# twosigma/Cook

Measured on AMD Instinct MI355X. Metric: match-cycles/sec at 1M pending x 50k offers, higher is better.
Workload: dtype f64

## Files before the change

### cook_amd/csrc/rank_host.hpp

```cpp

template <class T, class Load>
void seg_scan(cook_engine* e, const char* tag, Load load, const uint8_t* head, unsigned n, T* out, ScanTmp<T>& tmp) {
  if (n == 0) return;
  const unsigned nb = div_up(n, SS_TILE);
  tmp.agg.ensure(nb);
  tmp.carry.ensure(nb);
  tmp.first_head.ensure(nb);
  KM<seg_scan_local<T, Load>, SS_THREADS>(e, tag, nb, load, head, n, out, tmp.agg.ptr(), tmp.first_head.ptr());
  if (nb > 1 && nb <= (unsigned)SS_THREADS) {
    KM<seg_scan_propagate_fused<T>, SS_THREADS>(e, "seg_scan_propagate", nb, out, n, (const SegAgg<T>*)tmp.agg.ptr(), (const unsigned*)tmp.first_head.ptr());
  } else if (nb > 1) {
    KM<seg_scan_blocksums<T>, SS_THREADS>(e, "seg_scan_blocksums", 1, (const SegAgg<T>*)tmp.agg.ptr(), nb, tmp.carry.ptr());
    KM<seg_scan_propagate<T>, SS_THREADS>(e, "seg_scan_propagate", nb, out, n, (const SegAgg<T>*)tmp.carry.ptr(), (const unsigned*)tmp.first_head.ptr());
  }
}

template <int IPL>
static void radix_pass_t(cook_engine* e, const uint64_t* key, const uint32_t* in, uint32_t* out, unsigned n, unsigned shift, bool fused,
                         DArr<uint32_t>& hist) {
  const unsigned nb = div_up(n, rs_tile(IPL));
  hist.ensure((size_t)256 * nb);
  KM<radix_hist<IPL>, RS_THREADS>(e, "radix_hist", nb, key, in, n, shift, nb, fused ? 1u : 0u, hist.ptr());
  if (!fused) KM<excl_scan_u32_single, SCAN1_THREADS>(e, "radix_scan", 1, hist.ptr(), 256u * nb, (uint32_t*)nullptr);
  KM<radix_scatter<IPL>, RS_THREADS>(e, "radix_scatter", nb, key, in, out, n, shift, nb, fused ? 1u : 0u, (const uint32_t*)hist.ptr());
}
void radix_pass(cook_engine* e, const uint64_t* key, const uint32_t* in, uint32_t* out, unsigned n, unsigned shift, DArr<uint32_t>& hist) {
  if (div_up(n, rs_tile(RS_IPL_SMALL)) <= RS_FUSED_BLOCKS) radix_pass_t<RS_IPL_SMALL>(e, key, in, out, n, shift, true, hist);
  else radix_pass_t<RS_IPL_LARGE>(e, key, in, out, n, shift, div_up(n, rs_tile(RS_IPL_LARGE)) <= RS_FUSED_BLOCKS_LARGE, hist);
}
uint32_t* radix_sort_masked(cook_engine* e, const uint64_t* key, unsigned long long mask, const uint32_t* cur, uint32_t* a,
                            uint32_t* b, unsigned n, DArr<uint32_t>* hist = nullptr) {
  const uint32_t* in = cur;
  uint32_t* last = const_cast<uint32_t*>(cur);
  while (mask) {
    const unsigned shift = (unsigned)__builtin_ctzll(mask);
    uint32_t* out = (in == a) ? b : a;
    radix_pass(e, key, in, out, n, shift, hist ? *hist : e->hist);
    in = out;
    last = out;
    mask = shift + 8 >= 64 ? 0ull : mask & ~((1ull << (shift + 8)) - 1ull);
  }
  return last;
}

COOK_KERNEL void iota_u32(uint32_t* p, unsigned n) {
  const unsigned i = blockIdx.x * blockDim.x + threadIdx.x;
  if (i < n) p[i] = i;
}

void rank_stage(cook_engine* e, const cook_tasks* t, const cook_users* u) {
  if (!t || !u) e->fail(COOK_E_INVALID, "cook_rank_stage: null tasks/users");
  const unsigned N = t->n, U = u->n;
  if (N && (!t->cpus || !t->mem || !t->user || !t->priority || !t->start_ms || !t->task_id || !t->job_id || !t->pending))
    e->fail(COOK_E_INVALID, "cook_rank_stage: a required task array is NULL");
  if (U == 0 && N) e->fail(COOK_E_INVALID, "cook_rank_stage: no users");
  unsigned np = 0;
  std::vector<uint32_t> pend_ord(N ? N : 1);
  for (unsigned i = 0; i < N; ++i) {
    if (t->user[i] >= U) e->fail(COOK_E_INVALID, "cook_rank_stage: user id out of range");
    pend_ord[i] = np;
    np += t->pending[i] ? 1u : 0u;
  }
  e->rank_staged = false, e->pool_usage_known = false, e->rank_done = false;
  e->N = N;
  e->U = U;
  e->n_pending = np;
  e->has_gpus = t->gpus != nullptr;
  h2d(e, e->t_cpus, t->cpus, N);
  h2d(e, e->t_mem, t->mem, N);
  if (t->gpus) h2d(e, e->t_gpus, t->gpus, N);
  h2d(e, e->t_user, t->user, N);
  h2d(e, e->t_prio, t->priority, N);
  h2d(e, e->t_start, t->start_ms, N);
// ... 365 lines not shown
```

### cook_amd/csrc/sort.hpp

```cpp
#pragma once
#include "common.hpp"

constexpr int RS_THREADS = 256;
constexpr int RS_WAVES = RS_THREADS / COOK_WAVE;
constexpr int RS_IPL_LARGE = 16;
constexpr int RS_IPL_SMALL = 8;
constexpr unsigned RS_FUSED_BLOCKS = COOK_SHAPE(128, 2);
constexpr unsigned RS_FUSED_BLOCKS_LARGE = COOK_SHAPE(512, 3);
constexpr unsigned rs_tile(int ipl) { return (unsigned)(RS_WAVES * COOK_WAVE * ipl); }

static __device__ __forceinline__ unsigned rs_digit(const uint64_t* __restrict__ key, const uint32_t* __restrict__ perm_in,
                                                    unsigned i, unsigned shift) {
  const unsigned src = perm_in ? perm_in[i] : i;
  return (unsigned)(key[src] >> shift) & 0xFFu;
}

template <int IPL>
COOK_KERNEL void radix_hist(const uint64_t* __restrict__ key, const uint32_t* __restrict__ perm_in,
                                                         unsigned n, unsigned shift, unsigned nblocks, unsigned fused,
                                                         uint32_t* __restrict__ hist) {
  __shared__ unsigned h[256];
  h[threadIdx.x] = 0;
  __syncthreads();
  const unsigned base = blockIdx.x * rs_tile(IPL);
// ... 43 lines not shown
      for (int q = 0; q < SCAN1_IPT; ++q) tot += v[s][q];
      unsigned inc = tot;
      for (unsigned d = 1; d < COOK_WAVE; d <<= 1) {
        const unsigned t = __shfl_up(inc, d, COOK_WAVE);
        if (lane >= d) inc += t;
      }
      if (lane == COOK_WAVE - 1) wsum[s & 1][w] = inc;
      __syncthreads();
      unsigned wbase = 0, all = 0;
      for (unsigned k = 0; k < SCAN1_THREADS / COOK_WAVE; ++k) {
        const unsigned x = wsum[s & 1][k];
        wbase += k < w ? x : 0u;
        all += x;
      }
      unsigned run = carry + wbase + inc - tot;
      unsigned o[SCAN1_IPT];
#pragma unroll
      for (int q = 0; q < SCAN1_IPT; ++q) {
        o[q] = run;
        run += v[s][q];
      }
      if (i0 + SCAN1_IPT <= len) {
        *reinterpret_cast<uint4*>(data + i0) = uint4{o[0], o[1], o[2], o[3]};
        *reinterpret_cast<uint4*>(data + i0 + 4) = uint4{o[4], o[5], o[6], o[7]};
      } else {
#pragma unroll
        for (int q = 0; q < SCAN1_IPT; ++q)
          if (i0 + q < len) data[i0 + q] = o[q];
      }
      carry += all;
    }
  }
  if (total_out && threadIdx.x == 0) *total_out = carry;
}

template <int IPL>
COOK_KERNEL void radix_scatter(const uint64_t* __restrict__ key, const uint32_t* __restrict__ perm_in,
                                                            uint32_t* __restrict__ perm_out, unsigned n, unsigned shift,
                                                            unsigned nblocks, unsigned fused, const uint32_t* __restrict__ hist) {
  __shared__ unsigned whist[RS_WAVES][256];
  __shared__ unsigned wtot[RS_WAVES];
  __shared__ uint4 s_tot[RS_WAVES][COOK_WAVE], s_bel[RS_WAVES][COOK_WAVE];
  const unsigned lane = lane_id(), w = wave_id();
  for (int k = 0; k < RS_WAVES; ++k) whist[k][threadIdx.x] = 0;
  unsigned below = 0, total = 0;
  if (fused) {
    uint4 tot{0u, 0u, 0u, 0u}, bel{0u, 0u, 0u, 0u};
#pragma unroll 8
    for (unsigned t = w; t < nblocks; t += RS_WAVES) {
      const uint4 v = *reinterpret_cast<const uint4*>(hist + (size_t)t * 256u + 4u * lane);
      tot.x += v.x, tot.y += v.y, tot.z += v.z, tot.w += v.w;
      if (t < blockIdx.x) bel.x += v.x, bel.y += v.y, bel.z += v.z, bel.w += v.w;
    }
    s_tot[w][lane] = tot;
    s_bel[w][lane] = bel;
  }
  __syncthreads();
  if (fused) {
    const unsigned* pt = reinterpret_cast<const unsigned*>(&s_tot[0][0]);
    const unsigned* pb = reinterpret_cast<const unsigned*>(&s_bel[0][0]);
    for (int k = 0; k < RS_WAVES; ++k) {
      total += pt[k * 256 + threadIdx.x];
      below += pb[k * 256 + threadIdx.x];
    }
  }
  const unsigned wbase = blockIdx.x * rs_tile(IPL) + w * (COOK_WAVE * IPL);
// ... 2 lines not shown
  for (int k = 0; k < IPL; ++k) {
    const unsigned i = wbase + k * COOK_WAVE + lane;
    src[k] = i < n ? (perm_in ? perm_in[i] : i) : 0xFFFFFFFFu;
  }
#pragma unroll
  for (int k = 0; k < IPL; ++k) dg[k] = src[k] != 0xFFFFFFFFu ? (unsigned)(key[src[k]] >> shift) & 0xFFu : 0u;
#pragma unroll
  for (int k = 0; k < IPL; ++k)
    if (src[k] != 0xFFFFFFFFu) atomicAdd(&whist[w][dg[k]], 1u);
  if (fused) {
    unsigned inc = total;
    for (unsigned d = 1; d < COOK_WAVE; d <<= 1) {
      const unsigned t = __shfl_up(inc, d, COOK_WAVE);
      if (lane >= d) inc += t;
    }
    if (lane == COOK_WAVE - 1) wtot[w] = inc;
    __syncthreads();
    unsigned before = 0;
    for (unsigned k = 0; k < (unsigned)RS_WAVES; ++k) before += k < w ? wtot[k] : 0u;
    below += before + inc - total;
  } else {
    __syncthreads();
    below = hist[threadIdx.x * nblocks + blockIdx.x];
  }
  {
    unsigned base = below;
    for (int k = 0; k < RS_WAVES; ++k) {
      const unsigned t = whist[k][threadIdx.x];
      whist[k][threadIdx.x] = base;
      base += t;
    }
  }
  __syncthreads();
  const unsigned long long lt = lanemask_lt();
#pragma unroll
  for (int k = 0; k < IPL; ++k) {
    const bool valid = src[k] != 0xFFFFFFFFu;
    const unsigned d = dg[k];
    unsigned long long peers = __ballot(valid);
    for (int b = 0; b < 8; ++b) {
      const unsigned long long m = __ballot(valid && ((d >> b) & 1u));
      peers &= ((d >> b) & 1u) ? m : ~m;
    }
    unsigned slot = 0;
    if (valid) slot = whist[w][d];
    wave_sync();
    if (valid) {
      const unsigned rank = (unsigned)__popcll(peers & lt);
      if (rank == 0) whist[w][d] = slot + (unsigned)__popcll(peers);
      perm_out[slot + rank] = src[k];
    }
    wave_sync();
  }
}

COOK_KERNEL void radix_varying_bits(const uint64_t* __restrict__ key, unsigned n,
                                                          unsigned long long* __restrict__ out_mask, unsigned nblk) {
  const uint64_t k0 = key[0];
  unsigned long long m = 0;
  for (unsigned i = blockIdx.x * blockDim.x + threadIdx.x; i < n; i += nblk * blockDim.x) m |= key[i] ^ k0;
  for (int d = 32; d >= 1; d >>= 1) m |= __shfl_xor(m, d, COOK_WAVE);
  __shared__ unsigned long long s_m[256 / COOK_WAVE];
  if (lane_id() == 0) s_m[wave_id()] = m;
  __syncthreads();
  if (threadIdx.x == 0) {
    unsigned long long b = 0ull;
    for (unsigned w = 0; w < blockDim.x / COOK_WAVE; ++w) b |= s_m[w];
    if (b) atomicOr(out_mask, b);
  }
}
```

### cook_amd/csrc/classfit_walk.hpp

```cpp
#pragma once
#if defined(CF_PROF) && !defined(CF_STATS)
#define CF_STATS 1
#endif
#ifdef CF_STATS
#define CF_STAT(x) x
#define CF_TICKS() cook_ticks()
#else
#define CF_STAT(x) ((void)0)
#define CF_TICKS() 0ull
#endif
#ifdef CF_PROF
#define CF_PROF_T(x) const unsigned long long x = __builtin_readcyclecounter()
#define CF_PROF_ADD(i, d) prof[i] += (unsigned long long)(d)
#else
#define CF_PROF_T(x) ((void)0)
#define CF_PROF_ADD(i, d) ((void)0)
#endif

#ifndef CF_AHEAD
#define CF_AHEAD 10
#endif
constexpr unsigned CF_BOARD = CF_AHEAD;
#ifndef CF_SLOTS_N
#define CF_SLOTS_N 12
// ... 23 lines not shown
  uint32_t ofc, ofm, nfc, nfm, pad0, pad1;
};
struct CfPost {
  double fa;
  uint32_t w0;
  uint32_t pos;
  uint32_t fc, fm, cls, aux;
};
struct CfJobU {
  unsigned c, m, kind, L, n_eq, n_nov, grouped, grp, eq0, eq1, nov0, nov1;
};
struct CfLds {
  CfFree* fcm;
  uint16_t* cid;
  CfEnt* board;
  CfLog* log;
  uint32_t* ctrl;
  uint64_t* attr8;
  uint16_t *goff, *gcnt, *gids;
  CfJob* ring;
  CfPost* post2;
  CfClass* cls;
  uint32_t* pw;
  uint32_t* aw;
  uint32_t* gk;
  uint32_t* ovt;
  uint32_t* ovl;
  uint32_t* ckept;
  uint32_t* misc;
  const uint32_t* t;
  const uint32_t* envw;
};

static __device__ __forceinline__ unsigned cf_level_of(const uint32_t* t, uint32_t fc) {
  unsigned n = 0;
#pragma unroll
  for (int i = 0; i < CF_LV; ++i) n += fc >= t[i] ? 1u : 0u;
  return n;
}
struct CfLv8 {
  uint32_t v0, v1, v2, v3, v4, v5, v6, v7;
};
#define CF_FOR8(F) F(0) F(1) F(2) F(3) F(4) F(5) F(6) F(7)
static __device__ __forceinline__ uint32_t cf_lv_get(const CfLv8& a, unsigned i) {
  const bool b0 = (i & 1u) != 0u, b1 = (i & 2u) != 0u, b2 = (i & 4u) != 0u;
  const uint32_t r01 = b0 ? a.v1 : a.v0, r23 = b0 ? a.v3 : a.v2, r45 = b0 ? a.v5 : a.v4, r67 = b0 ? a.v7 : a.v6;
  const uint32_t r03 = b1 ? r23 : r01, r47 = b1 ? r67 : r45;
  return b2 ? r47 : r03;
}
struct CfChunkLane {
  unsigned cls, kind, pos0, n, Tc, Tm;
  unsigned long long dE;
  double hTc, hTm;
  CfLv8 lv, la;
};

static __device__ __forceinline__ void cf_setup_chunks(const CfClass* cls, unsigned nc, unsigned lw, unsigned lane, CfChunkLane& c, unsigned& nch_wave) {
  c.cls = 0xFFu, c.kind = 0xFEu, c.pos0 = 0u, c.n = 0u, c.Tc = 1u, c.Tm = 1u, c.dE = 0ull, c.hTc = 0.0, c.hTm = 0.0;
  unsigned acc = 0;
  for (unsigned ci = 0; ci < nc; ++ci) {
    const CfClass& cl = cls[ci];
    if (cl.wave != lw) continue;
    const unsigned nch = (cl.n + 63u) / 64u;
    if (lane >= acc && lane < acc + nch) {
      const unsigned x = lane - acc;
      c.cls = ci, c.kind = cl.kind, c.pos0 = cl.off + 64u * x, c.n = cf_min(64u, cl.n - 64u * x), c.Tc = cl.Tc, c.Tm = cl.Tm, c.dE = cl.dE, c.hTc = cl.hTc, c.hTm = cl.hTm;
    }
    acc += nch;
  }
  nch_wave = acc;
}

static __device__ __forceinline__ void cf_tighten(const CfLds& S, unsigned lane, unsigned ch, CfChunkLane& c) {
  const uint32_t* t = S.t;
  const unsigned pos0 = (unsigned)wave_read_lane((int)c.pos0, (int)ch), n = (unsigned)wave_read_lane((int)c.n, (int)ch);
  const bool in = lane < n;
  const CfFree f = S.fcm[pos0 + lane];
  const uint32_t cid = S.cid[pos0 + lane];
  const unsigned nl = in ? cf_level_of(t, f.c) : 0u;
  const bool free_host = !(cid & CF_OCC);
#define CF_TI_A(i) unsigned a##i = nl > (unsigned)i ? f.m + 1u : 0u;
#define CF_TI_R(i) unsigned r##i = (nl > (unsigned)i && free_host) ? f.m + 1u : 0u;
  CF_FOR8(CF_TI_A)
  CF_FOR8(CF_TI_R)
#undef CF_TI_A
#undef CF_TI_R
  wave_max8_u32(a0, a1, a2, a3, a4, a5, a6, a7);
  wave_max8_u32(r0, r1, r2, r3, r4, r5, r6, r7);
#define CF_TI_S(i) \
  if (lane == ch) c.la.v##i = a##i, c.lv.v##i = r##i;
  CF_FOR8(CF_TI_S)
#undef CF_TI_S
}
static __device__ __forceinline__ void cf_wave_tables(const CfLds& S, unsigned lw, unsigned lane, const CfChunkLane& c, unsigned kinds, unsigned n_kind) {
#define CF_TB_P(i) unsigned p##i = c.kind == 0u ? c.lv.v##i : 0u;
#define CF_TB_A(i) unsigned a##i = c.kind < 0xFEu ? c.la.v##i : 0u;
  CF_FOR8(CF_TB_P)
  CF_FOR8(CF_TB_A)
#undef CF_TB_P
#undef CF_TB_A
  wave_max8_u32(p0, p1, p2, p3, p4, p5, p6, p7);
  wave_max8_u32(a0, a1, a2, a3, a4, a5, a6, a7);
#define CF_TB_S(i) \
  if (lane == 0) S.pw[lw * CF_LV + i] = p##i, S.aw[lw * CF_LV + i] = a##i;
  CF_FOR8(CF_TB_S)
#undef CF_TB_S
  for (unsigned k = 1; k < n_kind; ++k) {
    if (!((kinds >> k) & 1u)) continue;
#define CF_TB_G(i) unsigned g##i = c.kind == k ? c.lv.v##i : 0u;
    CF_FOR8(CF_TB_G)
#undef CF_TB_G
    wave_max8_u32(g0, g1, g2, g3, g4, g5, g6, g7);
#define CF_TB_GS(i) \
  if (lane == 0) S.gk[k * CF_LV + i] = g##i;
    CF_FOR8(CF_TB_GS)
#undef CF_TB_GS
  }
}

static __device__ __forceinline__ bool cf_cons_ok(const CfLds& S, const CfJobU& J, unsigned id, bool active) {
  bool ok = true;
  if (J.n_eq) {
    const uint64_t a8 = S.attr8[active ? id : 0u];
#pragma unroll
    for (unsigned q = 0; q < 4u; ++q) {
      const unsigned e = ((q < 2u ? J.eq0 : J.eq1) >> (16u * (q & 1u))) & 0xFFFFu;
      if (q < J.n_eq) ok = ok && (unsigned)((a8 >> (8u * (e >> 8))) & 255ull) == (e & 255u);
    }
  }
  if (J.n_nov) {
#pragma unroll
    for (unsigned q = 0; q < 4u; ++q) {
      const unsigned h = ((q < 2u ? J.nov0 : J.nov1) >> (16u * (q & 1u))) & 0xFFFFu;
      if (q < J.n_nov) ok = ok && id != h;
    }
  }
  if (J.grouped) {
    const unsigned g0 = S.goff[J.grp], gn = ld_wg(&S.gcnt[J.grp]);
    for (unsigned x = 0; x < gn; ++x) ok = ok && id != (unsigned)S.gids[g0 + x];
  }
  return ok;
}
static __device__ __forceinline__ double cf_literal(unsigned Tc, unsigned Tm, unsigned fc, unsigned fm, unsigned jc, unsigned jm, double sc, double sm) {
  const double A = (double)(Tc - fc) * sc, Bm = (double)(Tm - fm) * sm, c = (double)jc * sc, m = (double)jm * sm;
  return ((A + c) / ((double)Tc * sc) + (Bm + m) / ((double)Tm * sm)) / 2.0;
}

struct CfAns {
  bool have, amb;
  unsigned pos, ch, cid, fc, fm, cls;
  double fa;
};
static __device__ __forceinline__ void cf_class_answer(const CfLds& S, const CfJobU& J, unsigned lane, CfChunkLane& c, CfAns& out, unsigned& scans,
                                                       unsigned& tightened) {
  out.have = false, out.amb = false, out.pos = 0u, out.ch = 0u, out.cid = 0u, out.fc = 0u, out.fm = 0u, out.cls = 0u, out.fa = 0.0;
  const uint32_t lvL = cf_lv_get(c.lv, J.L);
  unsigned long long m = __ballot(c.kind == J.kind && lvL > J.m);
  while (m) {
    const unsigned ch = (unsigned)__ffsll(m) - 1u;
    ++scans;
    const unsigned pos0 = (unsigned)wave_read_lane((int)c.pos0, (int)ch), n = (unsigned)wave_read_lane((int)c.n, (int)ch);
    const unsigned q = pos0 + lane;
    const CfFree f = S.fcm[q];
    const uint32_t cid = S.cid[q];
    const bool room = lane < n && f.c >= J.c && f.m >= J.m && !(cid & CF_OCC);
    const bool ok = room && cf_cons_ok(S, J, cid & CF_IDMASK, room);
    const unsigned long long b = __ballot(ok);
    if (b == 0ull) {
      if (__ballot(room) == 0ull) {
        cf_tighten(S, lane, ch, c);
        ++tightened;
      }
      m &= ~(1ull << ch);
      continue;
    }
    const unsigned q0 = (unsigned)__ffsll(b) - 1u;
    const unsigned fc0 = (unsigned)wave_read_lane((int)f.c, (int)q0), fm0 = (unsigned)wave_read_lane((int)f.m, (int)q0), cid0 = (unsigned)wave_read_lane((int)cid, (int)q0);
    const unsigned cls = (unsigned)wave_read_lane((int)c.cls, (int)ch);
    m &= ~__ballot(c.cls == cls);
    const bool tie = (cid0 & CF_TIE) != 0u;
    const double hTc = wave_read_lane_f64(c.hTc, (int)ch), hTm = wave_read_lane_f64(c.hTm, (int)ch);
    const double f0 = 1.0 - ((double)(fc0 - J.c) * hTc + (double)(fm0 - J.m) * hTm);
    if (!out.have || f0 > out.fa + CF_BAND) out.amb = tie;
    else if (f0 >= out.fa - CF_BAND) out.amb = true;
    if (!out.have || f0 > out.fa) out.fa = f0, out.cid = cid0 & CF_IDMASK, out.pos = pos0 + q0, out.fc = fc0, out.fm = fm0, out.cls = cls, out.ch = ch;
    out.have = true;
  }
}
static __device__ __forceinline__ void cf_class_query_exact(const CfLds& S, const CfJobU& J, unsigned lane, const CfChunkLane& c, double fmax, double sc, double sm, CfPost& out,
                                                            unsigned& scans) {
  out.fa = 0.0, out.w0 = 0u, out.pos = 0u, out.fc = 0u, out.fm = 0u, out.cls = 0u, out.aux = 0u;
  const uint32_t lvL = cf_lv_get(c.lv, J.L);
  unsigned long long m = __ballot(c.kind == J.kind && lvL > J.m);
  unsigned long long best_lit = 0ull;
  while (m) {
    const unsigned ch = (unsigned)__ffsll(m) - 1u;
    ++scans;
    const unsigned pos0 = (unsigned)wave_read_lane((int)c.pos0, (int)ch), n = (unsigned)wave_read_lane((int)c.n, (int)ch);
    const unsigned Tc = (unsigned)wave_read_lane((int)c.Tc, (int)ch), Tm = (unsigned)wave_read_lane((int)c.Tm, (int)ch), cls = (unsigned)wave_read_lane((int)c.cls, (int)ch);
    const double hTc = wave_read_lane_f64(c.hTc, (int)ch), hTm = wave_read_lane_f64(c.hTm, (int)ch);
    const unsigned q = pos0 + lane;
    const CfFree f = S.fcm[q];
    const uint32_t cid = S.cid[q];
// ... 48 lines not shown
  const bool has = lane == 0u || (lane < 7u && ((used_sets >> lane) & 1u));
  CfPost p;
  p.fa = 0.0, p.w0 = 0u, p.pos = p.fc = p.fm = p.cls = p.aux = 0u;
  if (has) p = posts[lane];
  const unsigned long long fb = (unsigned long long)__double_as_longlong(p.fa);
  const unsigned long long mx = wave_max_u64(fb);
  v.src = -1, v.id = v.pos = v.fc = v.fm = v.cls = v.aux = 0u;
  if (mx == 0ull) return v;
  const unsigned idmin = ~wave_max_u32((has && fb == mx) ? ~p.w0 : 0u);
  const unsigned wl = (unsigned)__ffsll(__ballot(has && fb == mx && p.w0 == idmin)) - 1u;
  v.src = (int)wl;
  v.id = (unsigned)wave_read_lane((int)p.w0, (int)wl), v.pos = (unsigned)wave_read_lane((int)p.pos, (int)wl), v.fc = (unsigned)wave_read_lane((int)p.fc, (int)wl),
  v.fm = (unsigned)wave_read_lane((int)p.fm, (int)wl), v.cls = (unsigned)wave_read_lane((int)p.cls, (int)wl), v.aux = (unsigned)wave_read_lane((int)p.aux, (int)wl);
  return v;
}
static __device__ __forceinline__ unsigned cf_poll(const uint32_t* p) { return (unsigned)wave_read_lane((int)ld_wg(p), 0); }
static __device__ __forceinline__ unsigned long long cf_below(unsigned s) { return (1ull << s) - 1ull; }

enum : unsigned { CFE_K = 0, CFE_M, CFE_NP, CFE_NCLS, CFE_NKIND, CFE_CMIN, CFE_MMIN, CFE_KC, CFE_KM, CFE_MINFC, CFE_MINFM, CFE_N = 12 };
constexpr float CF_BAND32 = 1.0f / 2097152.0f;

struct CfFixed {
  CfEnt board[CF_SLOTS * 8u];
  CfLog log[64];
  CfJob ring[2u * 64u];
  CfPost post2[8];
  CfClass cls[CF_MAXCLS];
  uint32_t pw[8u * CF_LV], aw[8u * CF_LV], gk[CF_MAXKIND * CF_LV], ovt[CF_LV];
  uint32_t ctrl[8];
  uint32_t ovl[192], ckept[3u * CF_MAXCLS], misc[CFX_N];
  uint32_t env_t[CF_LV], envw[CFE_N];
};
static_assert(sizeof(CfFixed) % 16 == 0, "the arrays behind it are 16-byte aligned");
#if COOK_HAS_ASM_WALK
#define CF_ASM_EPOCH_LIVE "57"
#include "classfit_asm.hpp"
static_assert(CF_EPOCH_AT == 58 && CF_OVL == 58, "classfit_asm.hpp: the overlay's size");
static_assert(offsetof(CfFixed, ctrl) == 13728 + (CF_SLOTS - 12) * 256 && offsetof(CfFixed, cls) == 9472 + (CF_SLOTS - 12) * 256 && sizeof(CfFixed) == 15280 + (CF_SLOTS - 12) * 256 && sizeof(CfClass) == 56 && offsetof(CfClass, hTc) == 32 &&
                  offsetof(CfClass, hTm) == 40 && offsetof(CfEnt, pos) == 8 && offsetof(CfEnt, cid) == 12 && offsetof(CfEnt, fc) == 16 && offsetof(CfEnt, fa) == 24 && sizeof(CfEnt) == 32 &&
                  sizeof(CfLog) == 32 && offsetof(CfLog, ofc) == 8,
              "classfit_asm.hpp: offsets of the LDS records");
typedef unsigned cf_u32x16 __attribute__((ext_vector_type(16)));
typedef unsigned cf_u32x8 __attribute__((ext_vector_type(8)));
typedef unsigned cf_u32x4 __attribute__((ext_vector_type(4)));
#endif

template <int ROLE>
static __device__ __forceinline__ void cf_walk_role(const CfLds& S, const MatchState& st, const CfBuf& b, const unsigned lw, const unsigned rep, const unsigned nrep,
                                                    const unsigned long long t_start) {
  constexpr bool is_decider = ROLE == 0, is_class_wave = ROLE == 1, is_books = ROLE == 2;
  const unsigned tid = threadIdx.x, lane = lane_id();
  CfCtl* ctl = b.ctl;
  const unsigned K = wave_uniform_u32(S.envw[CFE_K]), cmin = wave_uniform_u32(S.envw[CFE_CMIN]), mmin = wave_uniform_u32(S.envw[CFE_MMIN]);
  const uint32_t* t = S.t;
#define n_cls wave_uniform_u32(S.envw[CFE_NCLS])
#define n_kind wave_uniform_u32(S.envw[CFE_NKIND])
#define NP wave_uniform_u32(S.envw[CFE_NP])
  CfChunkLane c;
  unsigned nch_wave = 0;
  cf_setup_chunks(S.cls, n_cls, is_class_wave ? lw : 0xFFu, lane, c, nch_wave);
  c.lv = CfLv8{0u, 0u, 0u, 0u, 0u, 0u, 0u, 0u}, c.la = c.lv;
  unsigned my_kinds = 0;
  {
    const unsigned forw = is_class_wave ? lw : (is_decider && lane >= CF_OVL ? lane - CF_OVL + 1u : 0xFFu);
    for (unsigned ci = 0; ci < n_cls; ++ci)
      if (S.cls[ci].wave == forw && S.cls[ci].kind < 32u) my_kinds |= 1u << S.cls[ci].kind;
  }
  const unsigned wk = is_class_wave ? wave_uniform_u32(my_kinds) : 0u;
  unsigned one_cls = 0xFFFFFFFFu, u_off = 0, u_n = 0;
  double u_hTc = 0.0, u_hTm = 0.0;
  auto class_setup = [&] {
    unsigned cnt = 0, ci0 = 0;
    for (unsigned ci = 0; ci < n_cls; ++ci)
      if (S.cls[ci].wave == lw) ++cnt, ci0 = ci;
    one_cls = cnt == 1u ? ci0 : 0xFFFFFFFFu;
    const CfClass* cl = &S.cls[ci0];
    u_off = cl->off, u_n = cl->n, u_hTc = cl->hTc, u_hTm = cl->hTm;
  };
  if (is_class_wave) {
    class_setup();
    for (unsigned ch = 0; ch < nch_wave; ++ch) cf_tighten(S, lane, ch, c);
    if (rep == 0u && lw != 0u) cf_wave_tables(S, lw, lane, c, wk, n_kind);
  }
  CfOvLane o;
  o.valid = 0u, o.id = 0u, o.cls = 0u, o.fc = 0u, o.fm = 0u, o.hTc = 0.0, o.hTm = 0.0;
  unsigned nrm = 0, rm1 = 0xFFFFFFFFu, rm2 = 0xFFFFFFFFu;
  unsigned minfc_all = wave_uniform_u32(S.envw[CFE_MINFC]), minfm_all = wave_uniform_u32(S.envw[CFE_MINFM]);
  unsigned matched = 0, head = 0;
  unsigned jc = 0, jm = 0, jmeta = 0, jgrp = 0, jeq0 = 0, jeq1 = 0, jnov0 = 0, jnov1 = 0;
  int res = -1;
  unsigned long long b1m = 0ull;
  unsigned seen = 0, gen = 0;
  unsigned tight_applied = 0;
  bool bk_room0 = false, nx_room0 = false, nx_walk = false;
  unsigned st_scans = 0, st_exact = 0, st_open = 0, st_ovwin = 0, st_gpu = 0, st_epochs = 0, st_tight = 0, st_walked = 0, st_dead = 0, st_opendead = 0, st_spins = 0, st_flips = 0,
           st_rewinds = 0;
  unsigned long long tk_epoch = 0, tk_books = 0, tk_walk = 0, tk_phase1 = 0;
#ifdef CF_PROF
  unsigned long long prof[8] = {0, 0, 0, 0, 0, 0, 0, 0}, bnd0 = 0ull;
#endif
  auto job_of = [&](unsigned s) -> CfJobU {
    CfJobU J;
    J.c = (unsigned)wave_read_lane((int)jc, (int)s), J.m = (unsigned)wave_read_lane((int)jm, (int)s);
    const unsigned meta = (unsigned)wave_read_lane((int)jmeta, (int)s);
    J.kind = meta & 255u, J.L = (meta >> 8) & 15u, J.n_eq = (meta >> 12) & 15u, J.n_nov = (meta >> 16) & 15u, J.grouped = (meta >> 20) & 1u;
    J.grp = 0u, J.eq0 = J.eq1 = 0u, J.nov0 = J.nov1 = 0xFFFFFFFFu;
    if (meta >> 12) {
      J.grp = (unsigned)wave_read_lane((int)jgrp, (int)s), J.eq0 = (unsigned)wave_read_lane((int)jeq0, (int)s), J.eq1 = (unsigned)wave_read_lane((int)jeq1, (int)s),
      J.nov0 = (unsigned)wave_read_lane((int)jnov0, (int)s), J.nov1 = (unsigned)wave_read_lane((int)jnov1, (int)s);
    }
    return J;
  };
  auto tables_room_any = [&](unsigned L, unsigned m) -> bool {
    bool r = S.ovt[L] > m;
// ... 365 lines not shown
              }
            }
            bool done = false;
            if ((meta >> 12) == 0u && one_cls != 0xFFFFFFFFu) {
              const uint32_t lvL = cf_lv_get(c.lv, (meta >> 8) & 15u);
              const unsigned long long mk = cook_ballot(lvL > Jm);
              if (mk == 0ull) {
                st_lane0_b32(&e->tag, 0xFFFFFFFFu);
                st_lane0_b64(&e->pos, 0u, CF_ENT_NONE);
                st_lane0_b32(&e->tag, tag);
                done = true;
              } else {
                const unsigned ch = (unsigned)__ffsll(mk) - 1u;
                const unsigned pos0 = u_off + 64u * ch, n = u_n - 64u * ch;
                const CfFree f = S.fcm[pos0 + lane];
                const uint32_t cid = S.cid[pos0 + lane];
                const unsigned long long bb = cook_ballot((lane < n) & (f.c >= Jc) & (f.m >= Jm) & !(cid & CF_OCC));
                double fa = 1.0 - ((double)(f.c - Jc) * u_hTc + (double)(f.m - Jm) * u_hTm);
                if (bb != 0ull) {
                  const unsigned long long pm = bb & (0ull - bb);
                  const unsigned long long fb = (unsigned long long)__double_as_longlong(fa);
                  st_mask_b32(&e->tag, pm, 0xFFFFFFFFu);
                  st_mask_b128(&e->fc, pm, f.c, f.m, (unsigned)fb, (unsigned)(fb >> 32));
                  st_mask_b64(&e->pos, pm, (pos0 + lane) | ch << 16, (cid & CF_IDMASK) | one_cls << 16 | ((cid & CF_TIE) ? CF_ENT_AMB : 0u));
                  st_mask_b32(&e->tag, pm, tag);
                  done = true;
                  CF_STAT(++st_scans);
                }
              }
            }
            if (!done) {
              const CfJobU J = job_of(s);
              CfAns a;
              cf_class_answer(S, J, lane, c, a, st_scans, st_tight);
              const unsigned long long fb = (unsigned long long)__double_as_longlong(a.fa);
              st_lane0_b32(&e->tag, 0xFFFFFFFFu);
              st_lane0_b128(&e->fc, a.fc, a.fm, (unsigned)fb, (unsigned)(fb >> 32));
              st_lane0_b64(&e->pos, a.pos | a.ch << 16, a.have ? (a.cid | a.cls << 16 | (a.amb ? CF_ENT_AMB : 0u)) : CF_ENT_NONE);
              st_lane0_b32(&e->tag, tag);
            }
            CF_PROF_T(q2);
            CF_PROF_ADD(0, q1 - q0);
            CF_PROF_ADD(1, q2 - q1);
            CF_PROF_ADD(3, 1);
          };
          if (cnt != seen) {
            seen = cnt;
            CF_STAT(++st_rewinds);
            unsigned long long t2 = walkmask & ~cf_below(hw & 255u);
            unsigned o2 = hw >> 8, p2 = o2;
            while (p2 >= nrep) p2 -= nrep;
            for (; t2 != 0ull && o2 < cur_ord; t2 &= t2 - 1ull, ++o2, p2 = p2 + 1u == nrep ? 0u : p2 + 1u)
              if (p2 == rep && wk != 0u) answer((unsigned)__ffsll(t2) - 1u, o2, true);
          }
          if (cur_ord < (hw >> 8)) {
            todo = walkmask & ~cf_below(hw & 255u);
            cur_ord = hw >> 8;
            ph = cur_ord;
            while (ph >= nrep) ph -= nrep;
          }
          while (todo != 0ull && ph != rep) {
            todo &= todo - 1ull, ++cur_ord;
            ph = ph + 1u == nrep ? 0u : ph + 1u;
          }
          if (todo != 0ull && wk != 0u && cur_ord < (hw >> 8) + CF_BOARD) {
            const unsigned s = (unsigned)__ffsll(todo) - 1u;
            const unsigned ord = cur_ord;
// ... 185 lines not shown
              }
              for (; ip < li + ni; ++ip) {
                const unsigned np = noff + kept_before + (ip - li);
                if (lane == 0) st_agent(&b.scr_fc[np], S.ovl[3u * ip + 1u]), st_agent(&b.scr_fm[np], S.ovl[3u * ip + 2u]), st_agent(&b.scr_cid[np], S.ovl[3u * ip]);
              }
            }
            li += ni;
          }
        }
        drain_stores();
        EMU_SITE("classfit: epoch 3");
        __syncthreads();
        unsigned newM = 0;
        for (unsigned ci = 0; ci < n_cls; ++ci) newM += S.ckept[ci] + S.ckept[CF_MAXCLS + ci];
        for (unsigned q = tid; q < NP; q += CF_THREADS) {
          const bool inq = q < newM;
          const uint32_t fcq = inq ? ld_agent(&b.scr_fc[q]) : 0u, fmq = inq ? ld_agent(&b.scr_fm[q]) : 0u, cq = inq ? ld_agent(&b.scr_cid[q]) : 0u;
          bool tie = false;
          if (q + 1u < newM) {
            const uint32_t fcn = ld_agent(&b.scr_fc[q + 1u]), fmn = ld_agent(&b.scr_fm[q + 1u]), cn = ld_agent(&b.scr_cid[q + 1u]);
            if ((cn >> 16) == (cq >> 16)) {
              const CfClass* cl = &S.cls[cq >> 16];
              tie = (unsigned long long)fcn * cl->Tm + (unsigned long long)fmn * cl->Tc <= (unsigned long long)fcq * cl->Tm + (unsigned long long)fmq * cl->Tc + cl->dE;
            }
          }
          S.fcm[q] = CfFree{fcq, fmq}, S.cid[q] = inq ? (uint16_t)((cq & (CF_OCC | CF_IDMASK)) | (tie ? CF_TIE : 0u)) : (uint16_t)0u;
        }
        if (tid < n_cls) S.cls[tid].n = S.ckept[tid] + S.ckept[CF_MAXCLS + tid], S.cls[tid].off = S.ckept[2 * CF_MAXCLS + tid];
        EMU_SITE("classfit: epoch 4");
        __syncthreads();
        if (is_class_wave) {
          cf_setup_chunks(S.cls, n_cls, lw, lane, c, nch_wave);
          class_setup();
          for (unsigned ch = 0; ch < nch_wave; ++ch) cf_tighten(S, lane, ch, c);
          if (rep == 0u && lw != 0u) cf_wave_tables(S, lw, lane, c, wk, n_kind);
          tight_applied = st_tight;
        }
        if (tid == 0) S.misc[CFX_LOG_APPLIED] = S.misc[CFX_LOGN];
        tk_epoch += CF_TICKS() - te;
      }
      {
        ++gen;
        if (is_class_wave) {
          todo = walkmask & ~cf_below(s) & ~(1ull << s), cur_ord = (unsigned)__popcll(walkmask & cf_below(s)) + 1u;
          ph = cur_ord;
          while (ph >= nrep) ph -= nrep;
        }
      }
      if (tid == 0) st_wg(&S.ctrl[0], 0u);
      EMU_SITE("classfit: collective done");
      __syncthreads();
      if (is_class_wave) seen = cf_poll(&S.ctrl[1u + lw]);
    }
    tk_walk += CF_TICKS() - tw0;
    CF_PROF_T(cw1);
    CF_PROF_ADD(7, cw1 - cw0);
    const unsigned long long tp0 = CF_TICKS();
    if (is_decider && nw == 0u) decider_books(0u);
    if (nw != 0u) {
      if (is_class_wave) {
        const unsigned n_log = wave_uniform_u32(S.misc[CFX_LOGN]), a0 = wave_uniform_u32(S.misc[CFX_LOG_APPLIED]);
        const bool mine_e = lane >= a0 && lane < n_log && ((S.log[lane].info >> 8) & 15u) == lw;
        bool dirty = st_tight != tight_applied;
        for (unsigned long long mm = __ballot(mine_e); mm; mm &= mm - 1ull) {
          const unsigned x = (unsigned)__ffsll(mm) - 1u;
          const CfLog lg = S.log[x];
          const unsigned ch = (lg.info >> 12) & 255u;
          bool retable = ((lg.info >> 20) & 1u) != 0u;
          const unsigned nl = cf_level_of(t, lg.ofc);
#define CF_WAS_MAX(i) retable = retable || (__ballot(lane == ch && (unsigned)i < nl && c.lv.v##i == lg.ofm + 1u) != 0ull);
          CF_FOR8(CF_WAS_MAX)
#undef CF_WAS_MAX
          if (retable) {
            cf_tighten(S, lane, ch, c);
            ++st_tight;
            dirty = true;
          }
        }
        if (dirty && rep == 0u && lw != 0u) cf_wave_tables(S, lw, lane, c, wk, n_kind);
        tight_applied = st_tight;
      }
    }
    EMU_SITE("classfit: phase 2");
    __syncthreads();
    tk_phase1 += CF_TICKS() - tp0;
    if (is_books) {
      const unsigned long long tb0 = CF_TICKS();
      const unsigned long long mm = (unsigned long long)S.misc[CFX_MATCH_LO] | (unsigned long long)S.misc[CFX_MATCH_HI] << 32,
                               bb = (unsigned long long)S.misc[CFX_B1_LO] | (unsigned long long)S.misc[CFX_B1_HI] << 32;
      const unsigned n_log = wave_uniform_u32(S.misc[CFX_LOGN]);
      const CfJob j = S.ring[slot * 64u + (lane < bn ? lane : 0u)];
      const bool unm = lane < bn && !((mm >> lane) & 1ull);
      const unsigned L = (j.meta >> 8) & 15u;
      bool room = unm && tables_room_any(L, j.m);
      const bool flip = unm && !room && bk_room0 && n_log != 0u;
      if (__ballot(flip) != 0ull) {
        ++st_flips;
        for (unsigned x = 0; x < n_log; ++x) {
          const CfLog lg = S.log[x];
          if (flip && (lg.info & 255u) > lane && lg.ofc >= j.c && lg.ofm >= j.m) room = true;
        }
      }
      if (lane < bn && st.fail_code) {
        unsigned fail = 0u;
        if (unm) {
          fail = (((bb >> lane) & 1ull) ? 1u : 0u) | (room ? 2u : 0u);
          if (fail == 0u) fail = 8u;
        }
        st.fail_code[base + lane] = fail;
      }
// ... 198 lines not shown
```

Measured before the change: 21.69.

## Add onesweep radix sort with decoupled lookback and single multi-digit histogram

```diff
diff --git a/cook_amd/csrc/rank_host.hpp b/cook_amd/csrc/rank_host.hpp
--- a/cook_amd/csrc/rank_host.hpp
+++ b/cook_amd/csrc/rank_host.hpp
@@ -19,26 +19,70 @@
 static void radix_pass_t(cook_engine* e, const uint64_t* key, const uint32_t* in, uint32_t* out, unsigned n, unsigned shift, bool fused,
                          DArr<uint32_t>& hist) {
   const unsigned nb = div_up(n, rs_tile(IPL));
-  hist.ensure((size_t)256 * nb);
-  KM<radix_hist<IPL>, RS_THREADS>(e, "radix_hist", nb, key, in, n, shift, nb, fused ? 1u : 0u, hist.ptr());
-  if (!fused) KM<excl_scan_u32_single, SCAN1_THREADS>(e, "radix_scan", 1, hist.ptr(), 256u * nb, (uint32_t*)nullptr);
-  KM<radix_scatter<IPL>, RS_THREADS>(e, "radix_scatter", nb, key, in, out, n, shift, nb, fused ? 1u : 0u, (const uint32_t*)hist.ptr());
-}
-void radix_pass(cook_engine* e, const uint64_t* key, const uint32_t* in, uint32_t* out, unsigned n, unsigned shift, DArr<uint32_t>& hist) {
-  if (div_up(n, rs_tile(RS_IPL_SMALL)) <= RS_FUSED_BLOCKS) radix_pass_t<RS_IPL_SMALL>(e, key, in, out, n, shift, true, hist);
-  else radix_pass_t<RS_IPL_LARGE>(e, key, in, out, n, shift, div_up(n, rs_tile(RS_IPL_LARGE)) <= RS_FUSED_BLOCKS_LARGE, hist);
+  uint32_t* h = hist.ptr() + RS1_OFF_STATUS;
+  KM<radix_hist<IPL>, RS_THREADS>(e, "radix_hist", nb, key, in, n, shift, nb, fused ? 1u : 0u, h);
+  if (!fused) KM<excl_scan_u32_single, SCAN1_THREADS>(e, "radix_scan", 1, h, 256u * nb, (uint32_t*)nullptr);
+  KM<radix_scatter<IPL>, RS_THREADS>(e, "radix_scatter", nb, key, in, out, n, shift, nb, fused ? 1u : 0u, (const uint32_t*)h);
+}
+COOK_KERNEL void radix_scratch_clear(uint32_t* __restrict__ p, unsigned n) {
+  const unsigned i = blockIdx.x * blockDim.x + threadIdx.x;
+  if (i < n) p[i] = 0u;
+}
+static void radix_scratch(cook_engine* e, DArr<uint32_t>& hist, size_t words) {
+  const void* was = hist.b.p;
+  const size_t cap = hist.b.cap;
+  hist.ensure(words);
+  if (hist.b.p != was || hist.b.cap != cap) KM<radix_scratch_clear, 256>(e, "radix_scratch_clear", div_up(RS1_OFF_BASE, 256), hist.ptr(), RS1_OFF_BASE);
+}
+template <int IPL>
+static void radix_onesweep_t(cook_engine* e, const uint64_t* key, const RadixDigits& dg, const uint32_t*& in, uint32_t*& last, uint32_t* a, uint32_t* b,
+                             unsigned n, DArr<uint32_t>& hist) {
+  const unsigned nb = div_up(n, rs_tile(IPL));
+  const size_t per_digit = (size_t)nb * 256u;
+  radix_scratch(e, hist, RS1_OFF_STATUS + dg.nd * per_digit);
+  uint32_t* h = hist.ptr();
+  const unsigned nblk = std::min(div_up(n, RH_TILE), RH_MAX_BLOCKS);
+  KM<radix_hist_digits, RH_THREADS>(e, "radix_hist_digits", nblk, key, n, dg, nblk, h + RS1_OFF_ACC, h + RS1_OFF_DONE, h + RS1_OFF_BASE, h + RS1_OFF_TICKET,
+      (unsigned)(RS1_OFF_STATUS - RS1_OFF_TICKET + dg.nd * per_digit));
+  for (unsigned q = 0; q < dg.nd; ++q) {
+    uint32_t* out = (in == a) ? b : a;
+    KM<radix_onesweep<IPL>, RS_THREADS>(e, "radix_onesweep", nb, key, in, out, n, (unsigned)dg.shift[q], (const uint32_t*)(h + RS1_OFF_BASE + q * 256u),
+        h + RS1_OFF_TICKET + q, h + RS1_OFF_STATUS + q * per_digit);
+    in = out;
+    last = out;
+  }
 }
 uint32_t* radix_sort_masked(cook_engine* e, const uint64_t* key, unsigned long long mask, const uint32_t* cur, uint32_t* a,
-                            uint32_t* b, unsigned n, DArr<uint32_t>* hist = nullptr) {
+                            uint32_t* b, unsigned n, DArr<uint32_t>* hist_opt = nullptr) {
+  DArr<uint32_t>& hist = hist_opt ? *hist_opt : e->hist;
   const uint32_t* in = cur;
   uint32_t* last = const_cast<uint32_t*>(cur);
-  while (mask) {
-    const unsigned shift = (unsigned)__builtin_ctzll(mask);
-    uint32_t* out = (in == a) ? b : a;
-    radix_pass(e, key, in, out, n, shift, hist ? *hist : e->hist);
-    in = out;
-    last = out;
-    mask = shift + 8 >= 64 ? 0ull : mask & ~((1ull << (shift + 8)) - 1ull);
+  RadixDigits dg{};
+  for (unsigned long long m = mask; m;) {
+    const unsigned shift = (unsigned)__builtin_ctzll(m);
+    dg.shift[dg.nd++] = (unsigned char)shift;
+    m = shift + 8 >= 64 ? 0ull : m & ~((1ull << (shift + 8)) - 1ull);
+  }
+  if (n == 0) {
+    for (unsigned q = 0; q < dg.nd; ++q) last = (last == a) ? b : a;
+    return last;
+  }
+  if (dg.nd == 0) return last;
+  static const bool onesweep = env_switch_on_unless_zero("COOK_RADIX_ONESWEEP");
+  if (onesweep && div_up(n, rs_tile(RS1_IPL_SMALL)) <= RS1_TILES_SMALL) {
+    radix_onesweep_t<RS1_IPL_SMALL>(e, key, dg, in, last, a, b, n, hist);
+  } else if (onesweep && div_up(n, rs_tile(RS1_IPL_LARGE)) <= RS1_TILES_LARGE) {
+    radix_onesweep_t<RS1_IPL_LARGE>(e, key, dg, in, last, a, b, n, hist);
+  } else {
+    const bool small = div_up(n, rs_tile(RS_IPL_SMALL)) <= RS_FUSED_BLOCKS;
+    radix_scratch(e, hist, RS1_OFF_STATUS + (size_t)256 * div_up(n, rs_tile(small ? RS_IPL_SMALL : RS_IPL_LARGE)));
+    for (unsigned q = 0; q < dg.nd; ++q) {
+      uint32_t* out = (in == a) ? b : a;
+      if (small) radix_pass_t<RS_IPL_SMALL>(e, key, in, out, n, (unsigned)dg.shift[q], true, hist);
+      else radix_pass_t<RS_IPL_LARGE>(e, key, in, out, n, (unsigned)dg.shift[q], div_up(n, rs_tile(RS_IPL_LARGE)) <= RS_FUSED_BLOCKS_LARGE, hist);
+      in = out;
+      last = out;
+    }
   }
   return last;
 }
diff --git a/cook_amd/csrc/sort.hpp b/cook_amd/csrc/sort.hpp
--- a/cook_amd/csrc/sort.hpp
+++ b/cook_amd/csrc/sort.hpp
@@ -99,6 +99,30 @@
     }
   }
   if (total_out && threadIdx.x == 0) *total_out = carry;
+}
+
+template <int IPL>
+static __device__ __forceinline__ void rs_place(const unsigned (&src)[IPL], const unsigned (&dg)[IPL], unsigned* whist_w, uint32_t* __restrict__ perm_out) {
+  const unsigned long long lt = lanemask_lt();
+#pragma unroll
+  for (int k = 0; k < IPL; ++k) {
+    const bool valid = src[k] != 0xFFFFFFFFu;
+    const unsigned d = dg[k];
+    unsigned long long peers = __ballot(valid);
+    for (int b = 0; b < 8; ++b) {
+      const unsigned long long m = __ballot(valid && ((d >> b) & 1u));
+      peers &= ((d >> b) & 1u) ? m : ~m;
+    }
+    unsigned slot = 0;
+    if (valid) slot = whist_w[d];
+    wave_sync();
+    if (valid) {
+      const unsigned rank = (unsigned)__popcll(peers & lt);
+      if (rank == 0) whist_w[d] = slot + (unsigned)__popcll(peers);
+      perm_out[slot + rank] = src[k];
+    }
+    wave_sync();
+  }
 }
 
 template <int IPL>
@@ -167,26 +191,131 @@
     }
   }
   __syncthreads();
-  const unsigned long long lt = lanemask_lt();
+  rs_place<IPL>(src, dg, whist[w], perm_out);
+}
+
+constexpr int RS1_IPL_SMALL = COOK_SHAPE(8, 1);
+constexpr int RS1_IPL_LARGE = COOK_SHAPE(16, 2);
+constexpr unsigned RS1_TILES_SMALL = COOK_SHAPE(128, 48);
+constexpr unsigned RS1_TILES_LARGE = COOK_SHAPE(512, 64);
+constexpr unsigned RS1_MAX_DIGITS = 8;
+constexpr unsigned RS1_EMPTY = 0u, RS1_AGGREGATE = 1u << 30, RS1_PREFIX = 2u << 30, RS1_COUNT = (1u << 30) - 1u;
+constexpr int RS1_LOOK = 16;
+constexpr unsigned RS1_OFF_ACC = 0, RS1_OFF_DONE = 8 * 256, RS1_OFF_BASE = RS1_OFF_DONE + 64, RS1_OFF_TICKET = RS1_OFF_BASE + 8 * 256,
+                   RS1_OFF_STATUS = RS1_OFF_TICKET + 64;
+constexpr int RH_THREADS = 256;
+constexpr unsigned RH_IPT = 8, RH_TILE = RH_THREADS * RH_IPT, RH_MAX_BLOCKS = 256;
+struct RadixDigits {
+  unsigned nd;
+  unsigned char shift[RS1_MAX_DIGITS];
+};
+
+COOK_KERNEL void radix_hist_digits(const uint64_t* __restrict__ key, unsigned n, RadixDigits dg, unsigned nblk, uint32_t* __restrict__ acc,
+                                   uint32_t* __restrict__ done, uint32_t* __restrict__ base, uint32_t* __restrict__ clr, unsigned nclr) {
+  __shared__ unsigned h[RS1_MAX_DIGITS][256];
+  __shared__ unsigned s_last, wtot[RH_THREADS / COOK_WAVE];
+  for (unsigned q = 0; q < RS1_MAX_DIGITS; ++q) h[q][threadIdx.x] = 0;
+  __syncthreads();
+  for (unsigned t0 = blockIdx.x * RH_TILE; t0 < n; t0 += nblk * RH_TILE) {
+    uint64_t k[RH_IPT];
+#pragma unroll
+    for (unsigned x = 0; x < RH_IPT; ++x) {
+      const unsigned i = t0 + x * RH_THREADS + threadIdx.x;
+      k[x] = i < n ? key[i] : 0ull;
+    }
+#pragma unroll
+    for (unsigned x = 0; x < RH_IPT; ++x)
+      if (t0 + x * RH_THREADS + threadIdx.x < n)
+        for (unsigned q = 0; q < dg.nd; ++q) atomicAdd(&h[q][(unsigned)(k[x] >> dg.shift[q]) & 0xFFu], 1u);
+  }
+  for (unsigned i = blockIdx.x * RH_THREADS + threadIdx.x; i < nclr; i += nblk * RH_THREADS) clr[i] = 0u;
+  __syncthreads();
+  for (unsigned q = 0; q < dg.nd; ++q) {
+    const unsigned v = h[q][threadIdx.x];
+    if (v) atomicAdd(&acc[q * 256u + threadIdx.x], v);
+  }
+  __threadfence();
+  __syncthreads();
+  if (threadIdx.x == 0) s_last = atomicAdd(done, 1u) == nblk - 1u ? 1u : 0u;
+  __syncthreads();
+  if (!s_last) return;
+  __threadfence();
+  const unsigned lane = lane_id(), w = wave_id();
+  for (unsigned q = 0; q < dg.nd; ++q) {
+    const unsigned total = atomicExch(&acc[q * 256u + threadIdx.x], 0u);
+    unsigned inc = total;
+    for (unsigned d = 1; d < COOK_WAVE; d <<= 1) {
+      const unsigned t = __shfl_up(inc, d, COOK_WAVE);
+      if (lane >= d) inc += t;
+    }
+    if (lane == COOK_WAVE - 1) wtot[w] = inc;
+    __syncthreads();
+    unsigned before = 0;
+    for (unsigned k = 0; k < (unsigned)(RH_THREADS / COOK_WAVE); ++k) before += k < w ? wtot[k] : 0u;
+    base[q * 256u + threadIdx.x] = before + inc - total;
+    __syncthreads();
+  }
+  if (threadIdx.x == 0) atomicExch(done, 0u);
+}
+
+template <int IPL>
+COOK_KERNEL void radix_onesweep(const uint64_t* __restrict__ key, const uint32_t* __restrict__ perm_in, uint32_t* __restrict__ perm_out, unsigned n,
+                                unsigned shift, const uint32_t* __restrict__ base, uint32_t* __restrict__ ticket, uint32_t* __restrict__ status) {
+  __shared__ unsigned whist[RS_WAVES][256];
+  __shared__ unsigned s_tile;
+  const unsigned lane = lane_id(), w = wave_id();
+  if (threadIdx.x == 0) s_tile = atomicAdd(ticket, 1u);
+  for (int k = 0; k < RS_WAVES; ++k) whist[k][threadIdx.x] = 0;
+  __syncthreads();
+  const unsigned tile = s_tile;
+  const unsigned wbase = tile * rs_tile(IPL) + w * (COOK_WAVE * IPL);
+  unsigned src[IPL], dg[IPL];
 #pragma unroll
   for (int k = 0; k < IPL; ++k) {
-    const bool valid = src[k] != 0xFFFFFFFFu;
-    const unsigned d = dg[k];
-    unsigned long long peers = __ballot(valid);
-    for (int b = 0; b < 8; ++b) {
-      const unsigned long long m = __ballot(valid && ((d >> b) & 1u));
-      peers &= ((d >> b) & 1u) ? m : ~m;
-    }
-    unsigned slot = 0;
-    if (valid) slot = whist[w][d];
-    wave_sync();
-    if (valid) {
-      const unsigned rank = (unsigned)__popcll(peers & lt);
-      if (rank == 0) whist[w][d] = slot + (unsigned)__popcll(peers);
-      perm_out[slot + rank] = src[k];
-    }
-    wave_sync();
-  }
+    const unsigned i = wbase + k * COOK_WAVE + lane;
+    src[k] = i < n ? (perm_in ? perm_in[i] : i) : 0xFFFFFFFFu;
+  }
+#pragma unroll
+  for (int k = 0; k < IPL; ++k) dg[k] = src[k] != 0xFFFFFFFFu ? (unsigned)(key[src[k]] >> shift) & 0xFFu : 0u;
+#pragma unroll
+  for (int k = 0; k < IPL; ++k)
+    if (src[k] != 0xFFFFFFFFu) atomicAdd(&whist[w][dg[k]], 1u);
+  __syncthreads();
+  {
+    unsigned count = 0;
+    for (int k = 0; k < RS_WAVES; ++k) count += whist[k][threadIdx.x];
+    uint32_t* mine = status + (size_t)tile * 256u + threadIdx.x;
+    st_agent(mine, (tile == 0 ? RS1_PREFIX : RS1_AGGREGATE) | count);
+    unsigned excl = 0;
+    unsigned t = tile;
+    bool found = tile == 0;
+    while (!found) {
+      unsigned v[RS1_LOOK];
+#pragma unroll
+      for (int q = 0; q < RS1_LOOK; ++q) v[q] = (unsigned)q < t ? ld_agent(mine - (size_t)(tile - t + 1u + (unsigned)q) * 256u) : RS1_PREFIX;
+#pragma unroll
+      for (int q = 0; q < RS1_LOOK; ++q) {
+        if (!found) {
+          while ((v[q] >> 30) == 0u) {
+            SPIN_PAUSE_FAR();
+            v[q] = ld_agent(mine - (size_t)(tile - t + 1u + (unsigned)q) * 256u);
+          }
+          excl += v[q] & RS1_COUNT;
+          found = (v[q] >> 30) == 2u;
+        }
+      }
+      t = t > (unsigned)RS1_LOOK ? t - (unsigned)RS1_LOOK : 0u;
+    }
+    if (tile != 0) st_agent(mine, RS1_PREFIX | (excl + count));
+    unsigned slot = base[threadIdx.x] + excl;
+    for (int k = 0; k < RS_WAVES; ++k) {
+      const unsigned c = whist[k][threadIdx.x];
+      whist[k][threadIdx.x] = slot;
+      slot += c;
+    }
+  }
+  __syncthreads();
+  rs_place<IPL>(src, dg, whist[w], perm_out);
 }
 
 COOK_KERNEL void radix_varying_bits(const uint64_t* __restrict__ key, unsigned n,
```

Result: no change. 21.58 (-0.5%).

## Hoist level thresholds into registers and batch stale-chunk detection across log entries

Applied to the files above, without the earlier changes.

```diff
diff --git a/cook_amd/csrc/classfit_walk.hpp b/cook_amd/csrc/classfit_walk.hpp
--- a/cook_amd/csrc/classfit_walk.hpp
+++ b/cook_amd/csrc/classfit_walk.hpp
@@ -79,16 +79,28 @@
   const uint32_t* envw;
 };
 
+struct CfLv8 {
+  uint32_t v0, v1, v2, v3, v4, v5, v6, v7;
+};
+#define CF_FOR8(F) F(0) F(1) F(2) F(3) F(4) F(5) F(6) F(7)
 static __device__ __forceinline__ unsigned cf_level_of(const uint32_t* t, uint32_t fc) {
   unsigned n = 0;
 #pragma unroll
   for (int i = 0; i < CF_LV; ++i) n += fc >= t[i] ? 1u : 0u;
   return n;
 }
-struct CfLv8 {
-  uint32_t v0, v1, v2, v3, v4, v5, v6, v7;
-};
-#define CF_FOR8(F) F(0) F(1) F(2) F(3) F(4) F(5) F(6) F(7)
+static_assert(CF_LV == 8, "CfLv8 holds the call's levels");
+static __device__ __forceinline__ CfLv8 cf_levels_load(const uint32_t* t) {
+  const uint32_t t0 = t[0], t1 = t[1], t2 = t[2], t3 = t[3], t4 = t[4], t5 = t[5], t6 = t[6], t7 = t[7];
+  return CfLv8{wave_uniform_u32(t0), wave_uniform_u32(t1), wave_uniform_u32(t2), wave_uniform_u32(t3), wave_uniform_u32(t4), wave_uniform_u32(t5), wave_uniform_u32(t6), wave_uniform_u32(t7)};
+}
+static __device__ __forceinline__ unsigned cf_level_of(const CfLv8& t, uint32_t fc) {
+  unsigned n = 0;
+#define CF_LO(i) n += fc >= t.v##i ? 1u : 0u;
+  CF_FOR8(CF_LO)
+#undef CF_LO
+  return n;
+}
 static __device__ __forceinline__ uint32_t cf_lv_get(const CfLv8& a, unsigned i) {
   const bool b0 = (i & 1u) != 0u, b1 = (i & 2u) != 0u, b2 = (i & 4u) != 0u;
   const uint32_t r01 = b0 ? a.v1 : a.v0, r23 = b0 ? a.v3 : a.v2, r45 = b0 ? a.v5 : a.v4, r67 = b0 ? a.v7 : a.v6;
@@ -118,8 +130,7 @@
   nch_wave = acc;
 }
 
-static __device__ __forceinline__ void cf_tighten(const CfLds& S, unsigned lane, unsigned ch, CfChunkLane& c) {
-  const uint32_t* t = S.t;
+static __device__ __forceinline__ void cf_tighten(const CfLds& S, const CfLv8& t, unsigned lane, unsigned ch, CfChunkLane& c) {
   const unsigned pos0 = (unsigned)wave_read_lane((int)c.pos0, (int)ch), n = (unsigned)wave_read_lane((int)c.n, (int)ch);
   const bool in = lane < n;
   const CfFree f = S.fcm[pos0 + lane];
@@ -148,21 +159,17 @@
 #undef CF_TB_A
   wave_max8_u32(p0, p1, p2, p3, p4, p5, p6, p7);
   wave_max8_u32(a0, a1, a2, a3, a4, a5, a6, a7);
-#define CF_TB_S(i) \
-  if (lane == 0) S.pw[lw * CF_LV + i] = p##i, S.aw[lw * CF_LV + i] = a##i;
-  CF_FOR8(CF_TB_S)
-#undef CF_TB_S
+  st_lane0_b128(&S.pw[lw * CF_LV], p0, p1, p2, p3), st_lane0_b128(&S.pw[lw * CF_LV + 4], p4, p5, p6, p7);
+  st_lane0_b128(&S.aw[lw * CF_LV], a0, a1, a2, a3), st_lane0_b128(&S.aw[lw * CF_LV + 4], a4, a5, a6, a7);
   for (unsigned k = 1; k < n_kind; ++k) {
     if (!((kinds >> k) & 1u)) continue;
 #define CF_TB_G(i) unsigned g##i = c.kind == k ? c.lv.v##i : 0u;
     CF_FOR8(CF_TB_G)
 #undef CF_TB_G
     wave_max8_u32(g0, g1, g2, g3, g4, g5, g6, g7);
-#define CF_TB_GS(i) \
-  if (lane == 0) S.gk[k * CF_LV + i] = g##i;
-    CF_FOR8(CF_TB_GS)
-#undef CF_TB_GS
-  }
+    st_lane0_b128(&S.gk[k * CF_LV], g0, g1, g2, g3), st_lane0_b128(&S.gk[k * CF_LV + 4], g4, g5, g6, g7);
+  }
+  WAIT_LDS();
 }
 
 static __device__ __forceinline__ bool cf_cons_ok(const CfLds& S, const CfJobU& J, unsigned id, bool active) {
@@ -198,7 +205,7 @@
   unsigned pos, ch, cid, fc, fm, cls;
   double fa;
 };
-static __device__ __forceinline__ void cf_class_answer(const CfLds& S, const CfJobU& J, unsigned lane, CfChunkLane& c, CfAns& out, unsigned& scans,
+static __device__ __forceinline__ void cf_class_answer(const CfLds& S, const CfLv8& tl, const CfJobU& J, unsigned lane, CfChunkLane& c, CfAns& out, unsigned& scans,
                                                        unsigned& tightened) {
   out.have = false, out.amb = false, out.pos = 0u, out.ch = 0u, out.cid = 0u, out.fc = 0u, out.fm = 0u, out.cls = 0u, out.fa = 0.0;
   const uint32_t lvL = cf_lv_get(c.lv, J.L);
@@ -215,7 +222,7 @@
     const unsigned long long b = __ballot(ok);
     if (b == 0ull) {
       if (__ballot(room) == 0ull) {
-        cf_tighten(S, lane, ch, c);
+        cf_tighten(S, tl, lane, ch, c);
         ++tightened;
       }
       m &= ~(1ull << ch);
@@ -330,6 +337,7 @@
   uint32_t env_t[CF_LV], envw[CFE_N];
 };
 static_assert(sizeof(CfFixed) % 16 == 0, "the arrays behind it are 16-byte aligned");
+static_assert(offsetof(CfFixed, pw) % 16 == 0 && offsetof(CfFixed, aw) % 16 == 0 && offsetof(CfFixed, gk) % 16 == 0 && (CF_LV * 4) % 16 == 0, "cf_wave_tables stores the rows 16 bytes at a time");
 #if COOK_HAS_ASM_WALK
 #define CF_ASM_EPOCH_LIVE "57"
 #include "classfit_asm.hpp"
@@ -351,6 +359,8 @@
   CfCtl* ctl = b.ctl;
   const unsigned K = wave_uniform_u32(S.envw[CFE_K]), cmin = wave_uniform_u32(S.envw[CFE_CMIN]), mmin = wave_uniform_u32(S.envw[CFE_MMIN]);
   const uint32_t* t = S.t;
+  CfLv8 tl = CfLv8{0u, 0u, 0u, 0u, 0u, 0u, 0u, 0u};
+  if (is_class_wave) tl = cf_levels_load(t);
 #define n_cls wave_uniform_u32(S.envw[CFE_NCLS])
 #define n_kind wave_uniform_u32(S.envw[CFE_NKIND])
 #define NP wave_uniform_u32(S.envw[CFE_NP])
@@ -377,7 +387,7 @@
   };
   if (is_class_wave) {
     class_setup();
-    for (unsigned ch = 0; ch < nch_wave; ++ch) cf_tighten(S, lane, ch, c);
+    for (unsigned ch = 0; ch < nch_wave; ++ch) cf_tighten(S, tl, lane, ch, c);
     if (rep == 0u && lw != 0u) cf_wave_tables(S, lw, lane, c, wk, n_kind);
   }
   CfOvLane o;
@@ -809,7 +819,7 @@
             if (!done) {
               const CfJobU J = job_of(s);
               CfAns a;
-              cf_class_answer(S, J, lane, c, a, st_scans, st_tight);
+              cf_class_answer(S, tl, J, lane, c, a, st_scans, st_tight);
               const unsigned long long fb = (unsigned long long)__double_as_longlong(a.fa);
               st_lane0_b32(&e->tag, 0xFFFFFFFFu);
               st_lane0_b128(&e->fc, a.fc, a.fm, (unsigned)fb, (unsigned)(fb >> 32));
@@ -1061,7 +1071,7 @@
         if (is_class_wave) {
           cf_setup_chunks(S.cls, n_cls, lw, lane, c, nch_wave);
           class_setup();
-          for (unsigned ch = 0; ch < nch_wave; ++ch) cf_tighten(S, lane, ch, c);
+          for (unsigned ch = 0; ch < nch_wave; ++ch) cf_tighten(S, tl, lane, ch, c);
           if (rep == 0u && lw != 0u) cf_wave_tables(S, lw, lane, c, wk, n_kind);
           tight_applied = st_tight;
         }
@@ -1088,23 +1098,26 @@
     if (is_decider && nw == 0u) decider_books(0u);
     if (nw != 0u) {
       if (is_class_wave) {
+        const CfLog* lp = &S.log[lane];
+        const unsigned info = lp->info, ofc = lp->ofc, ofm = lp->ofm;
         const unsigned n_log = wave_uniform_u32(S.misc[CFX_LOGN]), a0 = wave_uniform_u32(S.misc[CFX_LOG_APPLIED]);
-        const bool mine_e = lane >= a0 && lane < n_log && ((S.log[lane].info >> 8) & 15u) == lw;
+        const bool mine = lane >= a0 && lane < n_log && ((info >> 8) & 15u) == lw;
+        const unsigned ch = (info >> 12) & 63u;
+        const unsigned nl = cf_level_of(tl, ofc);
+#define CF_LV_AT(i) const unsigned g##i = (unsigned)__shfl((int)c.lv.v##i, (int)ch, COOK_WAVE);
+        CF_FOR8(CF_LV_AT)
+#undef CF_LV_AT
+        bool was_max = ((info >> 20) & 1u) != 0u;
+#define CF_WAS_MAX(i) was_max = was_max | (((unsigned)i < nl) & (g##i == ofm + 1u));
+        CF_FOR8(CF_WAS_MAX)
+#undef CF_WAS_MAX
+        unsigned long long stale = 0ull;
+        for (unsigned long long fm = cook_ballot(mine & was_max); fm != 0ull; fm &= fm - 1ull) stale |= 1ull << (unsigned)wave_read_lane((int)ch, __ffsll(fm) - 1);
         bool dirty = st_tight != tight_applied;
-        for (unsigned long long mm = __ballot(mine_e); mm; mm &= mm - 1ull) {
-          const unsigned x = (unsigned)__ffsll(mm) - 1u;
-          const CfLog lg = S.log[x];
-          const unsigned ch = (lg.info >> 12) & 255u;
-          bool retable = ((lg.info >> 20) & 1u) != 0u;
-          const unsigned nl = cf_level_of(t, lg.ofc);
-#define CF_WAS_MAX(i) retable = retable || (__ballot(lane == ch && (unsigned)i < nl && c.lv.v##i == lg.ofm + 1u) != 0ull);
-          CF_FOR8(CF_WAS_MAX)
-#undef CF_WAS_MAX
-          if (retable) {
-            cf_tighten(S, lane, ch, c);
-            ++st_tight;
-            dirty = true;
-          }
+        for (; stale != 0ull; stale &= stale - 1ull) {
+          cf_tighten(S, tl, lane, (unsigned)__ffsll(stale) - 1u, c);
+          ++st_tight;
+          dirty = true;
         }
         if (dirty && rep == 0u && lw != 0u) cf_wave_tables(S, lw, lane, c, wk, n_kind);
         tight_applied = st_tight;
```

New measurement: 21.36 before, 22.25 after (median of 6 runs). 4.2% higher.
